# zkonduit/ezkl

Hardware: AMD Instinct MI355X
Metric: BN254 G1 MSM pts/s (2^20 points per GPU; NTT 2^22 elems/s in extra) (higher is better)
Workload: dtype u32x8 (254-bit modular integer, Montgomery); 1 GPU; configs[1]: standalone 2^20-point BN254 G1 MSM (uniform scalars, try-and-increment bases) + 2^22 scalar-field NTT per GPU; parallelism=points sharded across 1 rank(s); all_gather of 64-B partials + host fold

## Files before the change

### ezkl_amd/csrc/curve29.hpp

```cpp
#pragma once
#include "curve.hpp"
#include "field29.hpp"

namespace ezkl {

struct alignas(16) g1x29_t {
    f29_t x, y, zz, zzz;
};
struct g1a29_t {
    f29_t x, y;
};

EZ_D bool g1x29_is_id(const g1x29_t& p) { return Fq29::limbs_zero(p.zz); }
EZ_D g1x29_t g1x29_identity() {
    g1x29_t r;
    r.x = Fq29::zero(); r.y = Fq29::zero(); r.zz = Fq29::zero(); r.zzz = Fq29::zero();
    return r;
}
EZ_D g1a29_t g1a29_unpack(const g1a_t& p) {
    g1a29_t r;
    r.x = Fq29::unpack(p.x);
    r.y = Fq29::unpack(p.y);
    return r;
}
EZ_D bool g1a29_is_id(const g1a29_t& p) {
    uint32_t o = 0;
#pragma unroll
    for (int i = 0; i < 9; i++) o |= p.x.v[i] | p.y.v[i];
    return o == 0;
}

EZ_D g1x29_t g1x29_add_tail(const f29_t& u1, const f29_t& s1, const f29_t& p, const f29_t& r, const f29_t& zz, const f29_t& zzz) {
    g1x29_t o;
    const f29_t pp = Fq29::sqr(p);
    o.zz = Fq29::mul(zz, pp);
    const f29_t ppp = Fq29::mul(p, pp);
    o.zzz = Fq29::mul(zzz, ppp);
    const f29_t q = Fq29::mul(u1, pp);
#if !EZKL_FUSED_Y
    const f29_t e = Fq29::mul(s1, ppp);
#endif
    const f29_t rr = Fq29::sqr(r);
    const f29_t nq = Fq29::neg<1>(q);
    o.x = Fq29::normalize(Fq29::add(Fq29::add(rr, Fq29::neg<1>(ppp)), Fq29::add(nq, nq)));
    const f29_t d = Fq29::sub<3>(q, o.x);
#if EZKL_FUSED_Y
    o.y = Fq29::mul2add(r, d, Fq29::neg<3>(s1), ppp);
#else
    const f29_t rd = Fq29::mul(r, d);
    o.y = Fq29::normalize(Fq29::sub<1>(rd, e));
#endif
    return o;
}
EZ_D g1x29_t g1x29_double_affine(const g1a29_t& p) {
    const f29_t u = Fq29::add(p.y, p.y);
    const f29_t v = Fq29::sqr_cold(u);
    const f29_t w = Fq29::mul_cold(u, v);
    const f29_t s = Fq29::mul_cold(p.x, v);
    const f29_t xx = Fq29::sqr_cold(p.x);
    const f29_t m = Fq29::normalize(Fq29::add(Fq29::add(xx, xx), xx));
    const f29_t ns = Fq29::neg<1>(s);
    g1x29_t r;
    r.x = Fq29::normalize(Fq29::add(Fq29::sqr_cold(m), Fq29::add(ns, ns)));
    const f29_t d = Fq29::sub<3>(s, r.x);
    r.y = Fq29::normalize(Fq29::sub<1>(Fq29::mul_cold(m, d), Fq29::mul_cold(w, p.y)));
    r.zz = v;
    r.zzz = w;
    return r;
}
EZ_D g1x29_t g1x29_double(const g1x29_t& p) {
    if (g1x29_is_id(p)) return p;
    const f29_t u = Fq29::add(p.y, p.y);
    const f29_t v = Fq29::sqr_cold(u);
    const f29_t w = Fq29::mul_cold(u, v);
    const f29_t s = Fq29::mul_cold(p.x, v);
    const f29_t xx = Fq29::sqr_cold(p.x);
    const f29_t m = Fq29::normalize(Fq29::add(Fq29::add(xx, xx), xx));
    const f29_t ns = Fq29::neg<1>(s);
    g1x29_t r;
    r.x = Fq29::normalize(Fq29::add(Fq29::sqr_cold(m), Fq29::add(ns, ns)));
    const f29_t d = Fq29::sub<3>(s, r.x);
    r.y = Fq29::normalize(Fq29::sub<1>(Fq29::mul_cold(m, d), Fq29::mul_cold(w, p.y)));
    r.zz = Fq29::mul_cold(v, p.zz);
    r.zzz = Fq29::mul_cold(w, p.zzz);
    return r;
}
EZ_D g1x29_t g1x29_add_mixed(const g1x29_t& a, const g1a29_t& q, bool negate) {
    if (g1a29_is_id(q)) return a;
    const f29_t qy = negate ? Fq29::neg<0>(q.y) : q.y;
    if (g1x29_is_id(a)) {
        g1x29_t r;
        r.x = q.x;
        r.y = negate ? Fq29::normalize(qy) : q.y;
        r.zz = Fq29::one();
        r.zzz = Fq29::one();
        return r;
    }
    const f29_t u2 = Fq29::mul(q.x, a.zz);
    const f29_t s2 = Fq29::mul(qy, a.zzz);
    const f29_t p = Fq29::normalize(Fq29::sub<3>(u2, a.x));
    const f29_t r = Fq29::normalize(Fq29::sub<3>(s2, a.y));
    if (Fq29::is_zero_mod_p(p)) {
        if (Fq29::is_zero_mod_p(r)) {
            g1a29_t qq = q;
            if (negate) qq.y = Fq29::normalize(qy);
            return g1x29_double_affine(qq);
        }
        return g1x29_identity();
    }
    return g1x29_add_tail(a.x, a.y, p, r, a.zz, a.zzz);
}
EZ_D g1x29_t g1x29_add(const g1x29_t& a, const g1x29_t& b) {
    if (g1x29_is_id(a)) return b;
    if (g1x29_is_id(b)) return a;
    const f29_t u1 = Fq29::mul(a.x, b.zz), u2 = Fq29::mul(b.x, a.zz);
    const f29_t s1 = Fq29::mul(a.y, b.zzz), s2 = Fq29::mul(b.y, a.zzz);
    const f29_t p = Fq29::normalize(Fq29::sub<1>(u2, u1));
    const f29_t r = Fq29::normalize(Fq29::sub<1>(s2, s1));
    if (Fq29::is_zero_mod_p(p)) {
        if (Fq29::is_zero_mod_p(r)) return g1x29_double(a);
        return g1x29_identity();
    }
    return g1x29_add_tail(u1, s1, p, r, Fq29::mul(a.zz, b.zz), Fq29::mul(a.zzz, b.zzz));
}

EZ_D g1x29_t ld_g1x29(const g1x29_t* p) {
    g1x29_t r;
    const uint4* s = reinterpret_cast<const uint4*>(p);
    uint32_t* d = r.x.v;
#pragma unroll
    for (int k = 0; k < 9; k++) {
        const uint4 t = s[k];
        d[4 * k] = t.x; d[4 * k + 1] = t.y; d[4 * k + 2] = t.z; d[4 * k + 3] = t.w;
    }
    return r;
}
EZ_D void st_g1x29(g1x29_t* p, const g1x29_t& v) {
    uint4* d = reinterpret_cast<uint4*>(p);
    const uint32_t* s = v.x.v;
#pragma unroll
    for (int k = 0; k < 9; k++) d[k] = make_uint4(s[4 * k], s[4 * k + 1], s[4 * k + 2], s[4 * k + 3]);
}
EZ_D g1x29_t g1x29_shfl_xor(const g1x29_t& p, uint32_t mask) {
    g1x29_t r;
    const uint32_t* s = p.x.v;
    uint32_t* d = r.x.v;
#pragma unroll
    for (int k = 0; k < 36; k++) d[k] = __shfl_xor(s[k], mask);
    return r;
}
EZ_D g1x29_t g1x29_group_sum(g1x29_t acc, uint32_t width) {
#pragma unroll 1
    for (uint32_t s = width >> 1; s > 0; s >>= 1) acc = g1x29_add(acc, g1x29_shfl_xor(acc, s));
    return acc;
}

template <int S>
EZ_D f29_t f29_quad_bcast(const f29_t& x) {
    f29_t t = x, r;
    asm volatile("s_nop 1" : "+v"(t.v[0]), "+v"(t.v[1]), "+v"(t.v[2]), "+v"(t.v[3]), "+v"(t.v[4]), "+v"(t.v[5]), "+v"(t.v[6]), "+v"(t.v[7]), "+v"(t.v[8]));
#pragma unroll
    for (int i = 0; i < 9; i++) {
        r.v[i] = (uint32_t)__builtin_amdgcn_mov_dpp((int)t.v[i], S * 0x55, 0xf, 0xf, true);
        asm volatile("" : "+v"(r.v[i]));
    }
    return r;
}
EZ_D f29_t f29_sel(bool c, const f29_t& a, const f29_t& b) {
    f29_t r;
#pragma unroll
    for (int i = 0; i < 9; i++) r.v[i] = c ? a.v[i] : b.v[i];
    return r;
}
EZ_D f29_t f29_sel4(uint32_t q, const f29_t& x0, const f29_t& x1, const f29_t& x2, const f29_t& x3) {
    return f29_sel(q < 2, f29_sel(q == 0, x0, x1), f29_sel(q == 2, x2, x3));
}
template <int S>
EZ_D g1x29_t g1x29_quad_bcast(const g1x29_t& p) {
    g1x29_t r;
    r.x = f29_quad_bcast<S>(p.x); r.y = f29_quad_bcast<S>(p.y); r.zz = f29_quad_bcast<S>(p.zz); r.zzz = f29_quad_bcast<S>(p.zzz);
    return r;
}
EZ_D g1x29_t g1x29_add_quad(const g1x29_t& a, const g1x29_t& b, bool& special, uint32_t* dbg = nullptr) {
    const uint32_t q = threadIdx.x & 3u;
    g1x29_t o = a;
    special = __any(g1x29_is_id(a) || g1x29_is_id(b)) != 0;
    if (special) return o;
    const f29_t m1 = Fq29::mul(f29_sel4(q, a.x, b.x, a.y, b.y), f29_sel4(q, b.zz, a.zz, b.zzz, a.zzz));
    const f29_t u1 = f29_quad_bcast<0>(m1), s1 = f29_quad_bcast<2>(m1);
    const f29_t p = Fq29::normalize(Fq29::sub<1>(f29_quad_bcast<1>(m1), u1));
    const f29_t r = Fq29::normalize(Fq29::sub<1>(f29_quad_bcast<3>(m1), s1));
    special = __any(Fq29::is_zero_mod_p(p)) != 0;
    if (special) return o;
    const f29_t m2 = Fq29::mul(f29_sel4(q, a.zz, a.zzz, p, r), f29_sel4(q, b.zz, b.zzz, p, r));
    const f29_t pp = f29_quad_bcast<2>(m2), rr = f29_quad_bcast<3>(m2);
    const f29_t m3 = Fq29::mul(f29_sel(q == 1, p, f29_sel(q == 2, u1, m2)), pp);
    const f29_t ppp = f29_quad_bcast<1>(m3), qq = f29_quad_bcast<2>(m3);
    const f29_t nq = Fq29::neg<1>(qq);
    o.x = Fq29::normalize(Fq29::add(Fq29::add(rr, Fq29::neg<1>(ppp)), Fq29::add(nq, nq)));
    const f29_t d = Fq29::sub<3>(qq, o.x);
    const f29_t m4 = Fq29::mul(f29_sel(q == 2, r, f29_sel(q == 3, s1, m2)), f29_sel(q == 2, d, ppp));
    o.zz = f29_quad_bcast<0>(m3);
    o.zzz = f29_quad_bcast<1>(m4);
    o.y = Fq29::normalize(Fq29::sub<1>(f29_quad_bcast<2>(m4), f29_quad_bcast<3>(m4)));
    if (dbg) {
        const f29_t* t[14] = {&m1, &u1, &s1, &p, &r, &m2, &pp, &rr, &m3, &ppp, &qq, &o.x, &d, &m4};
        for (int k = 0; k < 14; k++)
            for (int i = 0; i < 9; i++) dbg[9 * k + i] = t[k]->v[i];
    }
    return o;
}
EZ_D g1x29_t g1x29_group_sum_coop(g1x29_t acc, uint32_t width) {
    const uint32_t nsteps = 3u + (31u - (uint32_t)__clz(width)) - 2u;
    g1x29_t t0 = acc;
#pragma unroll 1
    for (uint32_t k = 0; k < nsteps; k++) {
        g1x29_t a, b;
        if (k == 0) { a = g1x29_quad_bcast<0>(acc); b = g1x29_quad_bcast<1>(acc); }
        else if (k == 1) { a = g1x29_quad_bcast<2>(acc); b = g1x29_quad_bcast<3>(acc); }
        else if (k == 2) { a = t0; b = acc; }
        else { a = acc; b = g1x29_shfl_xor(acc, 4u << (k - 3u)); }
        bool special;
        g1x29_t r = g1x29_add_quad(a, b, special);
        if (special) r = g1x29_add(a, b);
        if (k == 0) t0 = r; else acc = r;
    }
    return acc;
}
EZ_D g1x29_t g1x29_block256_sum(g1x29_t acc, uint4* sh) {
    acc = g1x29_group_sum(acc, 64);
    if ((threadIdx.x & 63) == 0) {
        const uint32_t* s = acc.x.v;
#pragma unroll
        for (int k = 0; k < 9; k++) sh[k * 4 + (threadIdx.x >> 6)] = make_uint4(s[4 * k], s[4 * k + 1], s[4 * k + 2], s[4 * k + 3]);
    }
    __syncthreads();
    {
        uint32_t* d = acc.x.v;
#pragma unroll
        for (int k = 0; k < 9; k++) {
            const uint4 t = sh[k * 4 + (threadIdx.x & 3)];
            d[4 * k] = t.x; d[4 * k + 1] = t.y; d[4 * k + 2] = t.z; d[4 * k + 3] = t.w;
        }
    }
    __syncthreads();
    return g1x29_group_sum(acc, 4);
}
EZ_D g1x29_t g1x29_block256_sum_coop(const g1x29_t& acc0, uint4* sh) {
    g1x29_t acc = g1x29_group_sum_coop(acc0, 64);
    if ((threadIdx.x & 63) == 0) {
        const uint32_t* s = acc.x.v;
#pragma unroll
        for (int k = 0; k < 9; k++) sh[k * 4 + (threadIdx.x >> 6)] = make_uint4(s[4 * k], s[4 * k + 1], s[4 * k + 2], s[4 * k + 3]);
    }
    __syncthreads();
    {
        uint32_t* d = acc.x.v;
#pragma unroll
        for (int k = 0; k < 9; k++) {
            const uint4 t = sh[k * 4 + (threadIdx.x & 3)];
            d[4 * k] = t.x; d[4 * k + 1] = t.y; d[4 * k + 2] = t.z; d[4 * k + 3] = t.w;
        }
    }
    __syncthreads();
    return g1x29_group_sum(acc, 4);
}

EZ_D g1x29_t g1x29_block256_sum_coop_full(const g1x29_t& acc0, uint4* sh) {
    g1x29_t acc = g1x29_group_sum_coop(acc0, 64);
    if ((threadIdx.x & 63) == 0) {
        const uint32_t* s = acc.x.v;
#pragma unroll
        for (int k = 0; k < 9; k++) sh[k * 4 + (threadIdx.x >> 6)] = make_uint4(s[4 * k], s[4 * k + 1], s[4 * k + 2], s[4 * k + 3]);
    }
    __syncthreads();
    g1x29_t w;
    {
        uint32_t* d = w.x.v;
#pragma unroll
        for (int k = 0; k < 9; k++) {
            const uint4 t = sh[k * 4 + (threadIdx.x & 3)];
            d[4 * k] = t.x; d[4 * k + 1] = t.y; d[4 * k + 2] = t.z; d[4 * k + 3] = t.w;
        }
    }
    __syncthreads();
    return g1x29_group_sum_coop(w, 4);
}

}
```

### ezkl_amd/csrc/msm.hip

```cpp
#include "common.hpp"
#include <deque>
#include <thread>
#include <chrono>
#include "curve.hpp"
#include "curve29.hpp"
#include "host64.hpp"
#include <string.h>

namespace ezkl {

static constexpr uint32_t MSM_MAX_PART_BITS = 12;
static constexpr uint32_t MSM_SPAN_HEAVY = 16;
static constexpr uint32_t MSM_PART_STAGE = 13312;
static constexpr uint32_t MSM_BINSORT_STAGE = 15360;
static constexpr uint32_t MSM_HEAVY_CHUNK = 256;
static constexpr uint32_t MSM_DIGIT_E = 8;
static constexpr uint32_t MSM_LMIN = 8;
static constexpr uint32_t MSM_MAX_BIG = 64;
static constexpr uint32_t MSM_BIG_BLOCKS = 64;
static constexpr uint32_t MSM_BIG_ROWS = 8;

__device__ __forceinline__ uint32_t msm_part_of(uint32_t bucket, uint32_t NP) { return bucket ? 1u + (bucket & (NP - 1u)) : 0u; }
__device__ __forceinline__ uint32_t msm_lane_len(const uint32_t* offsets, uint32_t nb, uint32_t nlanes, uint32_t lmin) {
    const uint32_t l = (uint32_t)(((uint64_t)offsets[nb] + nlanes - 1) / nlanes);
// ... 203 lines not shown
    __syncthreads();
    return r;
}

__global__ __launch_bounds__(256) void msm_hist_kernel(const fe_t* scalars, size_t n, size_t per_block, WinPlan wp,
                                                       uint32_t LB, uint32_t NP, uint32_t* wg_hist, uint32_t* wg_cnt,
                                                       const fe_t* const* scal_list, uint32_t* zero_base, uint32_t zero_words, size_t bstride) {
    BOFF(); BSH(wg_hist); BSH(wg_cnt);
    if (scal_list) scalars = scal_list[blockIdx.z];
    if (zero_base) {
        BSH(zero_base);
        for (uint32_t i = blockIdx.x * 256 + threadIdx.x; i < zero_words; i += gridDim.x * 256) zero_base[i] = 0;
    }
    __shared__ uint32_t lh[(1u << MSM_MAX_PART_BITS) + 1];
    const uint32_t NQ = NP + 1;
    for (uint32_t p = threadIdx.x; p < NQ; p += 256) lh[p] = 0;
    __syncthreads();
    size_t lo = (size_t)blockIdx.x * per_block, hi = lo + per_block < n ? lo + per_block : n;
    for (size_t i0 = lo + threadIdx.x; i0 < hi; i0 += 4 * 256) {
        fe_t s[4];
        uint32_t neg[4], carry[4] = {0, 0, 0, 0};
#pragma unroll
        for (int q = 0; q < 4; q++) {
            const size_t i = i0 + (size_t)q * 256;
            if (i < hi) s[q] = msm_canon(scalars, i, neg[q]);
            else { s[q] = Fr::zero(); neg[q] = 0; }
        }
        for (uint32_t w = 0; w < wp.W; w++) {
            const uint32_t c = wp.width(w);
#pragma unroll
            for (int q = 0; q < 4; q++) {
                uint32_t bucket, sign;
                if (msm_digit_step(s[q], neg[q], c, carry[q], bucket, sign)) atomicAdd(&lh[msm_part_of(bucket, NP)], 1u);
            }
        }
    }
    __syncthreads();
    for (uint32_t p = threadIdx.x; p < NQ; p += 256) {
        wg_hist[(size_t)blockIdx.x * NQ + p] = lh[p];
        wg_cnt[(size_t)blockIdx.x * NQ + p] = lh[p];
    }
}
__global__ __launch_bounds__(1024) void msm_hist_scan_kernel(uint32_t* wg_hist, uint32_t G, uint32_t NP, uint32_t* part_count, size_t bstride) {
    BOFF(); BSH(wg_hist); BSH(part_count);
    __shared__ uint32_t sums[32][33];
    const uint32_t c = threadIdx.x & 31, j = threadIdx.x >> 5;
    const uint32_t p = blockIdx.x * 32 + c;
    const uint32_t chunk = (G + 31) / 32, g0 = j * chunk, g1 = g0 + chunk < G ? g0 + chunk : G;
    uint32_t s = 0;
    if (p < NP)
        for (uint32_t g = g0; g < g1; g++) s += wg_hist[(size_t)g * NP + p];
    sums[j][c] = s;
    __syncthreads();
    if (j == 0) {
        uint32_t run = 0;
        for (uint32_t q = 0; q < 32; q++) {
            uint32_t v = sums[q][c];
            sums[q][c] = run;
            run += v;
        }
        if (p < NP) part_count[p] = run;
    }
    __syncthreads();
    if (p < NP) {
        uint32_t run = sums[j][c];
        for (uint32_t g = g0; g < g1; g++) {
            uint32_t v = wg_hist[(size_t)g * NP + p];
            wg_hist[(size_t)g * NP + p] = run;
            run += v;
        }
    }
}
__device__ __forceinline__ void msm_part_scan_body(const uint32_t* part_count, uint32_t NQ, uint32_t* part_base, uint32_t* big_flag,
                                                   uint32_t* big_list, uint32_t* big_count, uint32_t* sh) {
    const uint32_t t = threadIdx.x;
    constexpr uint32_t PER = 5;
    uint32_t v[PER], sum = 0;
#pragma unroll
    for (uint32_t q = 0; q < PER; q++) {
        const uint32_t i = PER * t + q;
        v[q] = i < NQ ? part_count[i] : 0;
        sum += v[q];
    }
    uint32_t total;
    uint32_t run = msm_block_scan(sum, sh, total) - sum;
#pragma unroll
    for (uint32_t q = 0; q < PER; q++) {
        const uint32_t i = PER * t + q;
        if (i < NQ) part_base[i] = run;
        run += v[q];
    }
    if (t == 1023) part_base[NQ] = total;
#pragma unroll
    for (uint32_t q = 0; q < PER; q++) {
        const uint32_t i = PER * t + q;
        if (i == 0 || i >= NQ) continue;
        uint32_t slot = 0;
        if (v[q] > MSM_BINSORT_STAGE) {
            slot = atomicAdd(big_count, 1u);
            if (slot < MSM_MAX_BIG) big_list[slot] = i - 1;
            slot = slot < MSM_MAX_BIG ? slot + 1 : 0;
        }
        big_flag[i - 1] = slot;
    }
}
__global__ __launch_bounds__(1024) void msm_part_scan_kernel(const uint32_t* part_count, uint32_t NQ, uint32_t* part_base, uint32_t* big_flag,
                                                             uint32_t* big_list, uint32_t* big_count, size_t bstride) {
    BOFF(); BSH(part_count); BSH(part_base); BSH(big_flag); BSH(big_list); BSH(big_count);
    __shared__ uint32_t sh[1024];
    msm_part_scan_body(part_count, NQ, part_base, big_flag, big_list, big_count, sh);
}
__global__ __launch_bounds__(1024) void msm_partition_kernel(const fe_t* scalars, size_t n, size_t per_block, WinPlan wp,
                                                             uint32_t LB, uint32_t NP, size_t base_offset, size_t tab_stride,
                                                             const uint32_t* part_base, const uint32_t* wg_hist, const uint32_t* wg_cnt, uint2* entries,
                                                             uint32_t* vals, const fe_t* const* scal_list, size_t bstride) {
    BOFF(); BSH(part_base); BSH(wg_hist); BSH(wg_cnt); BSH(entries); BSH(vals);
    if (scal_list) scalars = scal_list[blockIdx.z];
    extern __shared__ uint32_t plds[];
    __shared__ uint32_t tsum[1024];
    const uint32_t NQ = NP + 1;
    uint32_t* start = plds;
    uint32_t* cursor = plds + (NQ + 1);
    uint32_t* gbase = plds + 2 * (NQ + 1);
    uint2* stage = reinterpret_cast<uint2*>(plds + 3 * (NQ + 1));
    const uint32_t t = threadIdx.x, T = blockDim.x;
    const uint32_t K = (NQ + T - 1) / T;
    uint32_t loc = 0;
    for (uint32_t q = 0; q < K; q++) {
        const uint32_t p = t * K + q;
        if (p < NQ) loc += wg_cnt[(size_t)blockIdx.x * NQ + p];
    }
    uint32_t total;
    uint32_t run = msm_block_scan(loc, tsum, total) - loc;
    for (uint32_t q = 0; q < K; q++) {
        const uint32_t p = t * K + q;
        if (p < NQ) {
            start[p] = run;
            cursor[p] = run;
            gbase[p] = part_base[p] + wg_hist[(size_t)blockIdx.x * NQ + p];
            run += wg_cnt[(size_t)blockIdx.x * NQ + p];
        }
    }
    __syncthreads();
    const size_t lo = (size_t)blockIdx.x * per_block, hi = lo + per_block < n ? lo + per_block : n;
    const size_t i = lo + t;
    if (i < hi) {
        uint32_t neg;
        fe_t s = msm_canon(scalars, i, neg);
        msm_foreach_digit(s, neg, wp, [&](uint32_t w, uint32_t bucket, uint32_t sign) {
            const uint32_t r = atomicAdd(&cursor[msm_part_of(bucket, NP)], 1u);
            stage[r] = make_uint2((uint32_t)(w * tab_stride + base_offset + i) | (sign << 31), bucket);
        });
    }
    __syncthreads();
    const uint32_t PB = 31 - __clz(NP);
    for (uint32_t idx = t; idx < total; idx += T) {
        const uint2 e = stage[idx];
        const uint32_t p = msm_part_of(e.y, NP);
        const uint32_t slot = gbase[p] + (idx - start[p]);
        if (p) entries[slot] = make_uint2(e.x, e.y >> PB);
        else vals[slot] = e.x;
    }
}
__device__ __forceinline__ uint32_t msm_wave_rank(uint32_t* cnt, uint32_t key) {
    const uint64_t active = __ballot(1);
    const uint32_t first = __builtin_amdgcn_readfirstlane(key);
    if (__ballot(key == first) == active) {
        const uint32_t rank = (uint32_t)__popcll(active & ((1ull << (threadIdx.x & 63u)) - 1ull));
        uint32_t base = 0;
        if (rank == 0) base = atomicAdd(&cnt[first], (uint32_t)__popcll(active));
        return (uint32_t)__builtin_amdgcn_readfirstlane(base) + rank;
    }
    return atomicAdd(&cnt[key], 1u);
}
__device__ __forceinline__ void msm_bins_scan(uint32_t* cnt, uint32_t* tsum, uint32_t nbins, uint32_t p, uint32_t beg, const uint32_t* part_base,
                                              bool emit, uint32_t* offsets, g1x29_t* buckets) {
    const uint32_t t = threadIdx.x;
    uint32_t loc[4], s = 0;
#pragma unroll
    for (int q = 0; q < 4; q++) {
        uint32_t j = t * 4 + q;
        loc[q] = j < nbins ? cnt[j] : 0;
        s += loc[q];
    }
    uint32_t total;
    uint32_t run = msm_block_scan(s, tsum, total) - s;
#pragma unroll
    for (int q = 0; q < 4; q++) {
        uint32_t j = t * 4 + q;
        if (j < nbins) {
            cnt[j] = run;
            if (emit) {
                const bool b0 = (p == 0 && j == 0);
                offsets[(size_t)p * nbins + j] = b0 ? part_base[0] : beg + run;
                if (b0 ? part_base[1] == part_base[0] : loc[q] == 0) st_f29(&buckets[(size_t)p * nbins + j].zz, Fq29::zero());
            }
        }
        run += loc[q];
    }
    __syncthreads();
}
__device__ __forceinline__ void msm_bigsort_count_body(const uint2* entries, const uint32_t* part_base, uint32_t LB, const uint32_t* big_list,
                                                       const uint32_t* big_count, uint32_t* bin_total, uint32_t* block_off, uint32_t* cnt, uint32_t bx,
                                                       uint32_t by, uint32_t rows);
__global__ __launch_bounds__(512) void msm_binsort_kernel(const uint2* entries, const uint32_t* part_base, uint32_t LB, uint32_t NP,
                                                          const uint32_t* big_flag, uint32_t* offsets, uint32_t* vals, g1x29_t* buckets,
                                                          const uint32_t* big_list, const uint32_t* big_count, uint32_t* bin_total, uint32_t* block_off,
                                                          size_t bstride) {
    BOFF(); BSH(entries); BSH(part_base); BSH(big_flag); BSH(offsets); BSH(vals); BSH(buckets);
    __shared__ uint32_t cnt[2048];
    __shared__ uint32_t tsum[512];
    extern __shared__ uint32_t stage[];
    if (blockIdx.x >= NP) {
        BSH(big_list); BSH(big_count); BSH(bin_total); BSH(block_off);
        const uint32_t w = blockIdx.x - NP;
        msm_bigsort_count_body(entries, part_base, LB, big_list, big_count, bin_total, block_off, cnt, w % MSM_BIG_BLOCKS, w / MSM_BIG_BLOCKS, MSM_BIG_ROWS);
        return;
    }
    const uint32_t p = blockIdx.x, t = threadIdx.x, nbins = 1u << LB;
    const uint32_t beg = part_base[p + 1], end = part_base[p + 2];
    if (p == NP - 1 && t == 0) offsets[(size_t)NP * nbins] = end;
    if (big_flag[p]) return;
    const bool staged = (end - beg) <= MSM_BINSORT_STAGE;
    for (uint32_t j = t; j < nbins; j += 512) cnt[j] = 0;
    __syncthreads();
    if (staged) {
        constexpr int PER = MSM_BINSORT_STAGE / 512;
        uint2 v[PER];
#pragma unroll
        for (int q = 0; q < PER; q++) {
            const uint32_t e = beg + t + (uint32_t)q * 512u;
            v[q] = e < end ? entries[e] : make_uint2(0u, 0xffffffffu);
        }
#pragma unroll
        for (int q = 0; q < PER; q++)
            if (v[q].y != 0xffffffffu) atomicAdd(&cnt[v[q].y], 1u);
        __syncthreads();
        msm_bins_scan(cnt, tsum, nbins, p, beg, part_base, true, offsets, buckets);
#pragma unroll
        for (int q = 0; q < PER; q++)
            if (v[q].y != 0xffffffffu) stage[atomicAdd(&cnt[v[q].y], 1u)] = v[q].x;
        __syncthreads();
        for (uint32_t i = t; i < end - beg; i += 512) vals[beg + i] = stage[i];
    } else {
        for (uint32_t e = beg + t; e < end; e += 512) (void)msm_wave_rank(cnt, entries[e].y);
        __syncthreads();
        msm_bins_scan(cnt, tsum, nbins, p, beg, part_base, true, offsets, buckets);
        for (uint32_t e = beg + t; e < end; e += 512) {
            const uint2 v = entries[e];
            vals[beg + msm_wave_rank(cnt, v.y)] = v.x;
        }
    }
}
__device__ __forceinline__ void msm_big_slice(uint32_t beg, uint32_t end, uint32_t& s0, uint32_t& s1, uint32_t bx) {
    const uint32_t chunk = (end - beg + MSM_BIG_BLOCKS - 1) / MSM_BIG_BLOCKS;
    s0 = beg + bx * chunk;
    s1 = s0 + chunk < end ? s0 + chunk : end;
    if (s0 > end) s0 = end;
}
__device__ __forceinline__ void msm_bigsort_count_body(const uint2* entries, const uint32_t* part_base, uint32_t LB, const uint32_t* big_list,
                                                       const uint32_t* big_count, uint32_t* bin_total, uint32_t* block_off, uint32_t* cnt, uint32_t bx,
                                                       uint32_t by, uint32_t rows) {
    const uint32_t t = threadIdx.x, nbins = 1u << LB;
    const uint32_t nbig = big_count[0] < MSM_MAX_BIG ? big_count[0] : MSM_MAX_BIG;
    for (uint32_t y = by; y < nbig; y += rows) {
        const uint32_t p = big_list[y];
        uint32_t s0, s1;
        msm_big_slice(part_base[p + 1], part_base[p + 2], s0, s1, bx);
        for (uint32_t j = t; j < nbins; j += 512) cnt[j] = 0;
        __syncthreads();
        for (uint32_t e = s0 + t; e < s1; e += 512) (void)msm_wave_rank(cnt, entries[e].y);
        __syncthreads();
        for (uint32_t j = t; j < nbins; j += 512)
            block_off[((size_t)y * MSM_BIG_BLOCKS + bx) * nbins + j] = cnt[j] ? atomicAdd(&bin_total[(size_t)y * nbins + j], cnt[j]) : 0u;
        __syncthreads();
    }
}
__global__ __launch_bounds__(512) void msm_bigsort_scatter_kernel(const uint2* entries, const uint32_t* part_base, uint32_t LB, const uint32_t* big_list,
                                                                  const uint32_t* big_count, const uint32_t* bin_total, const uint32_t* block_off,
                                                                  uint32_t* offsets, uint32_t* vals, g1x29_t* buckets, size_t bstride) {
    BOFF(); BSH(entries); BSH(part_base); BSH(big_list); BSH(big_count); BSH(bin_total); BSH(block_off); BSH(offsets); BSH(vals); BSH(buckets);
    __shared__ uint32_t cnt[2048];
    __shared__ uint32_t tsum[512];
    const uint32_t t = threadIdx.x, nbins = 1u << LB;
    const uint32_t nbig = big_count[0] < MSM_MAX_BIG ? big_count[0] : MSM_MAX_BIG;
    for (uint32_t y = blockIdx.y; y < nbig; y += gridDim.y) {
        const uint32_t p = big_list[y], beg = part_base[p + 1];
        uint32_t s0, s1;
        msm_big_slice(beg, part_base[p + 2], s0, s1, blockIdx.x);
        for (uint32_t j = t; j < nbins; j += 512) cnt[j] = bin_total[(size_t)y * nbins + j];
        __syncthreads();
        msm_bins_scan(cnt, tsum, nbins, p, beg, part_base, blockIdx.x == 0, offsets, buckets);
        const uint32_t* mine = block_off + ((size_t)y * MSM_BIG_BLOCKS + blockIdx.x) * nbins;
        for (uint32_t j = t; j < nbins; j += 512) cnt[j] += mine[j];
        __syncthreads();
        for (uint32_t e = s0 + t; e < s1; e += 512) {
            const uint2 v = entries[e];
            vals[beg + msm_wave_rank(cnt, v.y)] = v.x;
        }
        __syncthreads();
    }
}

struct MsmRec {
    g1a_t p;
    bool neg;
};
__device__ __forceinline__ MsmRec msm_fetch(const g1a_t* tab, uint32_t v) {
    MsmRec r;
    r.p = ld_g1a(tab + (v & 0x7fffffffu));
    r.neg = (v >> 31) != 0;
    return r;
}
__global__ __launch_bounds__(256, 3) void msm_accumulate_kernel(const g1a_t* tab, const uint32_t* offsets, const uint32_t* vals,
                                                             uint32_t nb, uint32_t nlanes, g1x29_t* buckets, g1x29_t* head, g1x29_t* tail,
                                                             uint32_t* lane_first, uint32_t lmin, size_t bstride) {
    BOFF(); BSH(offsets); BSH(vals); BSH(buckets); BSH(head); BSH(tail); BSH(lane_first);
    const uint32_t t = blockIdx.x * blockDim.x + threadIdx.x;
    const uint32_t total = offsets[nb], L = msm_lane_len(offsets, nb, nlanes, lmin);
    const uint64_t k0w = (uint64_t)t * L;
    if (k0w >= total) return;
    const uint32_t k0 = (uint32_t)k0w;
    const uint32_t k1 = (uint64_t)k0 + L < total ? k0 + L : total;
    uint32_t lo = 0, hi = nb;
    while (hi - lo > 1) {
        uint32_t mid = (lo + hi) >> 1;
        if (offsets[mid] <= k0) lo = mid; else hi = mid;
    }
    uint32_t b = lo, bin_end = offsets[b + 1];
    uint32_t end_next = offsets[b + 2 <= nb ? b + 2 : nb];
    lane_first[t] = b;
    bool started_before = offsets[b] < k0;
    g1x29_t acc = g1x29_identity();
    MsmRec nxt = msm_fetch(tab, vals[k0]);
    uint32_t vn = k0 + 1 < k1 ? vals[k0 + 1] : 0u;
    for (uint32_t k = k0; k < k1; k++) {
        if (k == bin_end) {
            if (started_before) st_g1x29(head + t, acc); else st_g1x29(buckets + b, acc);
            acc.zz = Fq29::zero();
            started_before = false;
            b++;
            bin_end = end_next;
            if (bin_end == k) {
                uint32_t probes = 1;
                while (bin_end == k && probes < 4) { b++; bin_end = offsets[b + 1]; probes++; }
                if (bin_end == k) {
                    uint32_t lo2 = b + 1, hi2 = nb;
                    while (hi2 - lo2 > 1) {
                        uint32_t mid = (lo2 + hi2) >> 1;
                        if (offsets[mid] <= k) lo2 = mid; else hi2 = mid;
                    }
                    b = lo2;
                    bin_end = offsets[b + 1];
                }
            }
            end_next = offsets[b + 2 <= nb ? b + 2 : nb];
        }
        const MsmRec cur = nxt;
        nxt = msm_fetch(tab, vn);
        vn = k + 2 < k1 ? vals[k + 2] : 0u;
        acc = g1x29_add_mixed(acc, g1a29_unpack(cur.p), cur.neg);
    }
    if (k1 == bin_end) {
        if (started_before) st_g1x29(head + t, acc); else st_g1x29(buckets + b, acc);
    } else {
        if (started_before) st_g1x29(head + t, acc); else st_g1x29(tail + t, acc);
    }
}
EZ_D g1x29_t g1x29_shfl_down(const g1x29_t& p, uint32_t d) {
    g1x29_t r;
    const uint32_t* s = p.x.v;
    uint32_t* o = r.x.v;
#pragma unroll
    for (int k = 0; k < 36; k++) o[k] = __shfl_down(s[k], d);
    return r;
}
__global__ __launch_bounds__(256) void msm_fixup_boundary_tree_kernel(const uint32_t* offsets, uint32_t nb, uint32_t nlanes,
                                                                      const uint32_t* lane_first, const g1x29_t* head, const g1x29_t* tail, g1x29_t* buckets,
                                                                      uint32_t* heavy_list, uint32_t* heavy_count, uint32_t* chunk_list, uint32_t lmin,
                                                                      uint32_t span_heavy, size_t bstride) {
    BOFF(); BSH(offsets); BSH(lane_first); BSH(head); BSH(tail); BSH(buckets); BSH(heavy_list); BSH(heavy_count); BSH(chunk_list);
    const uint32_t t = blockIdx.x * blockDim.x + threadIdx.x + 1;
    const uint32_t lane = threadIdx.x & 63u;
    const uint32_t L = msm_lane_len(offsets, nb, nlanes, lmin);
    const uint64_t k0 = (uint64_t)t * L;
    bool cut = t < nlanes && k0 < offsets[nb];
    uint32_t b = 0, t1 = 0, t2 = 0;
    if (cut) {
        b = lane_first[t];
        const uint32_t beg = offsets[b], end = offsets[b + 1];
        cut = beg < k0;
        t1 = beg / L; t2 = (end - 1) / L;
    }
    if (cut && t2 - t1 > span_heavy) {
        if (t == t1 + 1 && t2 - t1 > MSM_HEAVY_CHUNK) heavy_list[atomicAdd(heavy_count, 1u)] = b;
        if ((t - t1 - 1) % MSM_HEAVY_CHUNK == 0) chunk_list[atomicAdd(heavy_count + 1, 1u)] = t;
        cut = false;
    }
    const uint32_t wave_last = t + (63u - lane);
    const uint32_t run = cut ? (t2 < wave_last ? t2 : wave_last) - t + 1u : 0u;
    uint32_t longest = run;
#pragma unroll
    for (uint32_t o = 32; o > 0; o >>= 1) {
        const uint32_t m = __shfl_xor(longest, o);
        longest = m > longest ? m : longest;
    }
    if (longest == 0) return;
    if (longest <= 2) {
        if (!cut || t != t1 + 1) return;
        g1x29_t acc = g1x29_add(ld_g1x29(tail + t1), ld_g1x29(head + t));
        for (uint32_t u = t + 1; u <= t2; u++) acc = g1x29_add(acc, ld_g1x29(head + u));
        st_g1x29(buckets + b, acc);
        return;
    }
    g1x29_t v = cut ? ld_g1x29(head + t) : g1x29_identity();
    uint32_t have = cut ? 1u : 0u;
#pragma unroll 1
    for (uint32_t d = 1; d < longest; d <<= 1) {
        const g1x29_t w = g1x29_shfl_down(v, d);
        const uint32_t hw = __shfl_down(have, d);
        if (have == d && run > d) {
            v = g1x29_add(v, w);
            have += hw;
        }
    }
    if (!cut || t != t1 + 1) return;
    g1x29_t acc = g1x29_add(ld_g1x29(tail + t1), v);
    for (uint32_t u = t + run; u <= t2; u++) acc = g1x29_add(acc, ld_g1x29(head + u));
    st_g1x29(buckets + b, acc);
}
__global__ __launch_bounds__(256) void msm_fixup_heavy1_kernel(const uint32_t* offsets, uint32_t nb, uint32_t nlanes, const uint32_t* lane_first, g1x29_t* head,
                                                               const g1x29_t* tail, g1x29_t* buckets, const uint32_t* chunk_list, const uint32_t* counts, uint32_t lmin,
                                                               uint32_t coop, size_t bstride) {
    BOFF(); BSH(offsets); BSH(lane_first); BSH(head); BSH(tail); BSH(buckets); BSH(chunk_list); BSH(counts);
    const uint32_t nchunks = counts[1], L = msm_lane_len(offsets, nb, nlanes, lmin);
    const uint32_t wave = threadIdx.x >> 6, lane = threadIdx.x & 63u;
    for (uint32_t ci = blockIdx.x * 4u + wave; ci < nchunks; ci += gridDim.x * 4u) {
        const uint32_t start = chunk_list[ci], b = lane_first[start];
        const uint32_t t2 = (offsets[b + 1] - 1) / L;
        const uint32_t stop = start + MSM_HEAVY_CHUNK - 1 < t2 ? start + MSM_HEAVY_CHUNK - 1 : t2;
        const uint32_t t1 = offsets[b] / L;
        const bool whole = t2 - t1 <= MSM_HEAVY_CHUNK;
        g1x29_t acc = (whole && lane == 63u) ? ld_g1x29(tail + t1) : g1x29_identity();
        for (uint32_t t = start + lane; t <= stop; t += 64) acc = g1x29_add(acc, ld_g1x29(head + t));
        acc = coop ? g1x29_group_sum_coop(acc, 64) : g1x29_group_sum(acc, 64);
        if (lane == 0) st_g1x29(whole ? buckets + b : head + start, acc);
    }
}
__global__ __launch_bounds__(256) void msm_fixup_heavy2_kernel(const uint32_t* offsets, uint32_t nb, uint32_t nlanes, const g1x29_t* head, const g1x29_t* tail,
                                                               const uint32_t* heavy_list, const uint32_t* counts, g1x29_t* buckets, uint32_t lmin, uint32_t coop, size_t bstride) {
    BOFF(); BSH(offsets); BSH(head); BSH(tail); BSH(heavy_list); BSH(counts); BSH(buckets);
    const uint32_t L = msm_lane_len(offsets, nb, nlanes, lmin);
    const uint32_t wave = threadIdx.x >> 6, lane = threadIdx.x & 63u;
    for (uint32_t h = blockIdx.x * 4u + wave; h < counts[0]; h += gridDim.x * 4u) {
        const uint32_t b = heavy_list[h];
        const uint32_t t1 = offsets[b] / L, t2 = (offsets[b + 1] - 1) / L;
        g1x29_t acc = lane == 63u ? ld_g1x29(tail + t1) : g1x29_identity();
        for (uint32_t t = t1 + 1 + lane * MSM_HEAVY_CHUNK; t <= t2; t += 64 * MSM_HEAVY_CHUNK) acc = g1x29_add(acc, ld_g1x29(head + t));
        acc = coop ? g1x29_group_sum_coop(acc, 64) : g1x29_group_sum(acc, 64);
        if (lane == 0) st_g1x29(buckets + b, acc);
    }
}

struct ReduceGeom {
    uint32_t wA, wB, wC;
    uint32_t wsA, wsB, wsC;
    uint32_t EA, GA, ET, GT;
};
__global__ __launch_bounds__(256, 2) void msm_reduce1_kernel(const g1x29_t* buckets, ReduceGeom g, g1x29_t* partA, g1x29_t* partT, size_t bstride) {
    BOFF(); BSH(buckets); BSH(partA); BSH(partT);
    const uint32_t idx = blockIdx.x * blockDim.x + threadIdx.x;
    g1x29_t acc = g1x29_identity();
    if (blockIdx.y == 0) {
        if (idx >= (g.GA << g.wA)) return;
        const uint32_t dA = idx & ((1u << g.wA) - 1u), grp = idx >> g.wA;
        for (uint32_t e = 0; e < g.EA; e++) acc = g1x29_add(acc, ld_g1x29(buckets + ((((size_t)grp * g.EA + e) << g.wA) | dA)));
        st_g1x29(partA + (size_t)dA * g.GA + grp, acc);
    } else {
        const uint32_t nT = 1u << (g.wB + g.wC);
        if (idx >= nT * g.GT) return;
        const uint32_t grp = idx % g.GT, t = idx / g.GT;
        for (uint32_t e = 0; e < g.ET; e++) acc = g1x29_add(acc, ld_g1x29(buckets + (((size_t)t << g.wA) | (e * g.GT + grp))));
        st_g1x29(partT + (size_t)t * g.GT + grp, acc);
    }
}
__global__ __launch_bounds__(64) void msm_reduce2_kernel(const g1x29_t* partA, const g1x29_t* partT, ReduceGeom g, g1x29_t* SA, g1x29_t* T, uint32_t lanesA,
                                                         uint32_t lanesT, uint32_t blocksA, uint32_t coop, size_t bstride) {
    BOFF(); BSH(partA); BSH(partT); BSH(SA); BSH(T);
    const bool isA = blockIdx.x < blocksA;
    const uint32_t lanes = isA ? lanesA : lanesT, per = 64 / lanes;
    const uint32_t o = (isA ? blockIdx.x : blockIdx.x - blocksA) * per + threadIdx.x / lanes, j = threadIdx.x % lanes;
    const uint32_t nout = isA ? (1u << g.wA) : (1u << (g.wB + g.wC)), G = isA ? g.GA : g.GT;
    g1x29_t acc = g1x29_identity();
    if (o < nout) {
        const g1x29_t* src = (isA ? partA : partT) + (size_t)o * G;
        for (uint32_t i = j; i < G; i += lanes) acc = g1x29_add(acc, ld_g1x29(src + i));
    }
    acc = (coop && lanes >= 4) ? g1x29_group_sum_coop(acc, lanes) : g1x29_group_sum(acc, lanes);
    if (j == 0 && o < nout) st_g1x29((isA ? SA : T) + o, acc);
}
__global__ __launch_bounds__(256) void msm_planes_kernel(const g1x29_t* SA, const g1x29_t* T, ReduceGeom g, g1x29_t* planes, g1x29_t* planes_host, uint32_t coop,
                                                         size_t bstride) {
    BOFF(); BSH(SA); BSH(T); BSH(planes);
    __shared__ uint4 sh[9 * 4];
    uint32_t id = blockIdx.x, field = 0, j = 0;
    if (id > 0) {
        id -= 1;
        if (id < g.wA) { field = 1; j = id; }
        else if (id < g.wA + g.wB) { field = 2; j = id - g.wA; }
        else { field = 3; j = id - g.wA - g.wB; }
    }
    const uint32_t nA = 1u << g.wA, nT = 1u << (g.wB + g.wC);
    g1x29_t acc = g1x29_identity();
    auto with_bit = [](uint32_t k, uint32_t bit) { return ((k >> bit) << (bit + 1)) | (1u << bit) | (k & ((1u << bit) - 1u)); };
    if (field == 0) {
        for (uint32_t d = threadIdx.x; d < nA; d += 256) acc = g1x29_add(acc, ld_g1x29(SA + d));
    } else if (field == 1) {
        for (uint32_t k = threadIdx.x; k < nA / 2; k += 256) acc = g1x29_add(acc, ld_g1x29(SA + with_bit(k, j)));
    } else {
        const uint32_t sh_bits = field == 2 ? j : g.wB + j;
        for (uint32_t k = threadIdx.x; k < nT / 2; k += 256) acc = g1x29_add(acc, ld_g1x29(T + with_bit(k, sh_bits)));
    }
    acc = (coop & 8u) ? g1x29_block256_sum_coop_full(acc, sh) : coop ? g1x29_block256_sum_coop(acc, sh) : g1x29_block256_sum(acc, sh);
    if (threadIdx.x == 0) {
        const uint32_t ws = field == 1 ? g.wsA : field == 2 ? g.wsB : g.wsC;
        const uint32_t slot = field == 0 ? 0u : 1u + ws + j;
        st_g1x29(planes + slot, acc);
        if (planes_host) st_g1x29(planes_host + (size_t)blockIdx.z * 32 + slot, acc);
    }
}

static int table_build(Ctx* c, hipStream_t st, const Bases* b, bool wait) {
    MsmTable t;
    t.n = b->n;
    t.wp = pick_plan(b->n);
    if ((size_t)t.wp.W * t.n >= ((size_t)1 << 31)) return EZKL_ERR_UNSUPPORTED;
    EZ_HIP(hipMalloc(&t.tab, (size_t)t.wp.W * t.n * sizeof(g1a_t)));
    EZ_HIP(hipMemcpyAsync(t.tab, b->pts, t.n * sizeof(g1a_t), hipMemcpyDeviceToDevice, st));
    for (uint32_t w = 1; w < t.wp.W; w++)
        hipLaunchKernelGGL(msm_precompute_kernel, dim3(cdiv(t.n, 256)), dim3(256), 0, st, t.tab + (size_t)(w - 1) * t.n,
                           t.tab + (size_t)w * t.n, t.n, t.wp.width(w - 1));
    hipLaunchKernelGGL(msm_table_to_r261_kernel, dim3(cdiv((size_t)t.wp.W * t.n, 256)), dim3(256), 0, st, t.tab, (size_t)t.wp.W * t.n);
    EZ_HIP(hipGetLastError());
    EZ_HIP(hipEventCreateWithFlags(&t.ready, hipEventDisableTiming));
    EZ_HIP(hipEventRecord(t.ready, st));
    if (wait) {
        EZ_HIP(hipStreamSynchronize(st));
        t.synced = true;
    }
    g_tables[b] = t;
    return EZKL_OK;
}
static int table_get(Ctx* c, hipStream_t st, const Bases* b, MsmTable** out) {
    auto it = g_tables.find(b);
    if (it == g_tables.end()) {
        int rc = table_build(c, st, b, true);
        if (rc) return rc;
        it = g_tables.find(b);
    }
    if (!it->second.synced) {
        EZ_HIP(hipEventSynchronize(it->second.ready));
        it->second.synced = true;
    }
    *out = &it->second;
    return EZKL_OK;
}
int msm_table_prepare(Ctx* c, const Bases* b) {
    if (g_tables.count(b)) return EZKL_OK;
    if (!g_table_stream) EZ_HIP(hipStreamCreateWithFlags(&g_table_stream, hipStreamNonBlocking));
    return table_build(c, g_table_stream, b, false);
}
void msm_table_drop(const Bases* b) {
    auto it = g_tables.find(b);
    if (it != g_tables.end()) {
        if (it->second.ready) { (void)hipEventSynchronize(it->second.ready); (void)hipEventDestroy(it->second.ready); }
        (void)hipFree(it->second.tab);
        g_tables.erase(it);
    }
}

static constexpr size_t MSM_MAX_GROUP = 16;
static int slot_prepare(MsmSlot& sl, size_t bytes, size_t msms = 1) {
    if (!sl.st) {
        EZ_HIP(stream_create_prio(&sl.st, "EZKL_HIP_PRIO_MSM", 0));
        EZ_HIP(hipEventCreateWithFlags(&sl.done, hipEventDisableTiming));
        EZ_HIP(hipHostMalloc((void**)&sl.list_pinned, MSM_MAX_GROUP * sizeof(void*), hipHostMallocDefault));
    }
    if (msms > sl.pinned_msms) {
        if (sl.pinned) {
            EZ_HIP(hipStreamSynchronize(sl.st));
            EZ_HIP(hipHostFree(sl.pinned));
            sl.pinned = nullptr;
        }
        EZ_HIP(hipHostMalloc((void**)&sl.pinned, msms * 32 * sizeof(g1x29_t), hipHostMallocDefault));
        EZ_HIP(hipHostGetDevicePointer(&sl.pinned_dev, sl.pinned, 0));
        sl.pinned_msms = msms;
    }
    if (bytes > sl.scratch_bytes) {
        if (sl.scratch) {
            EZ_HIP(hipStreamSynchronize(sl.st));
            EZ_HIP(hipFree(sl.scratch));
            sl.scratch = nullptr;
            sl.scratch_bytes = 0;
        }
        size_t want = bytes + (bytes >> 4);
        EZ_HIP(hipMalloc((void**)&sl.scratch, want));
        sl.scratch_bytes = want;
    }
    return EZKL_OK;
}
static int msm_finish(MsmSlot& sl, void* out_host = nullptr, bool release = true) {
    if (!out_host) out_host = sl.out;
    EZ_HIP(hipEventSynchronize(sl.done));
    for (uint32_t j = 0; j < sl.count; j++) {
        const uint32_t* hp = sl.pinned + (size_t)j * 32 * 36;
        h64::xyzz acc = h64::identity();
        for (int k = (int)sl.bits - 1; k >= 0; k--) {
            acc = h64::dbl(acc);
            acc = h64::add(acc, h64::from_limbs29_point(hp + 36 * (1 + k)));
        }
        acc = h64::add(acc, h64::from_limbs29_point(hp));
        h64::aff r = h64::to_affine(acc);
        memcpy((uint8_t*)out_host + 64 * (size_t)j, &r, 64);
    }
    if (release) sl.busy = false;
    return EZKL_OK;
}

static size_t msm_group_size(const MsmTable* T, size_t n, bool small_scalars, size_t batch = 0) {
    if (const char* e = getenv("EZKL_MSM_GROUP")) {
        const int v = atoi(e);
        if (v >= 1 && v <= (int)MSM_MAX_GROUP) return (size_t)v;
    }
    (void)T; (void)n; (void)batch;
    if (small_scalars) {
        static const int small = [] { const char* e = getenv("EZKL_MSM_GROUP_SMALL"); const int v = e ? atoi(e) : 0; return v >= 1 && v <= (int)MSM_MAX_GROUP ? v : 6; }();
        return (size_t)small;
    }
    static const int big = [] { const char* e = getenv("EZKL_MSM_GROUP_BIG"); const int v = e ? atoi(e) : 0; return v >= 1 && v <= (int)MSM_MAX_GROUP ? v : 4; }();
    return (size_t)big;
}
static int msm_enqueue(Ctx* c, MsmSlot& sl, hipStream_t st, MsmTable* T, size_t base_offset, const fe_t* const* cols, size_t count, size_t n, bool timed) {
    int rc = EZKL_OK;
    if (count < 1 || count > MSM_MAX_GROUP) return EZKL_ERR_INVALID;
    const unsigned Z = (unsigned)count;
    const fe_t* scalars = cols[0];
    const WinPlan wp = T->wp;
    const uint32_t W = wp.W, bits = wp.cmax() - 1;
    const uint32_t nb = 1u << bits;
    const size_t npairs = n * W;
    uint32_t PB = bits < 10 ? bits : 10;
    while (PB < bits && PB < MSM_MAX_PART_BITS && (npairs >> PB) > (size_t)MSM_BINSORT_STAGE * 9 / 10) PB++;
    const uint32_t LB = bits - PB, NP = 1u << PB;
    int& acc_blocks_per_cu = msm_state().acc_blocks_per_cu;
    if (!acc_blocks_per_cu) {
        EZ_HIP(hipFuncSetAttribute((const void*)msm_binsort_kernel, hipFuncAttributeMaxDynamicSharedMemorySize, 96 * 1024));
        EZ_HIP(hipFuncSetAttribute((const void*)msm_partition_kernel, hipFuncAttributeMaxDynamicSharedMemorySize, 144 * 1024));
        EZ_HIP(hipOccupancyMaxActiveBlocksPerMultiprocessor(&acc_blocks_per_cu, msm_accumulate_kernel, 256, 0));
        if (acc_blocks_per_cu < 1) acc_blocks_per_cu = 1;
    }
    const size_t resident = (size_t)acc_blocks_per_cu * 256 * c->num_cus;
    const size_t load = npairs >> bits, per_lane = load * 9 / 10 > 40 ? load * 9 / 10 : 40;
    size_t rounds = npairs / (resident * per_lane);
    if (rounds < 1) rounds = 1;
    uint32_t L = (uint32_t)((npairs + resident * rounds - 1) / (resident * rounds));
    if (L < 8) L = 8;
    if (const char* e = getenv("EZKL_MSM_L")) {
        const int v = atoi(e);
        if (v > 0 && v < (1 << 20)) L = (uint32_t)v;
    }
// ... 642 lines not shown
```

Before: 807.3 million pts/s.

## Spill bucket zz/zzz to LDS and prefetch bases via global_load_lds in accumulate

The MSM accumulate kernel now keeps only the affine-like x/y accumulator in registers and moves the zz/zzz coordinates into per-thread LDS slots, read and written with inline ds_read/ds_write asm. The next base point is prefetched straight into LDS with global_load_lds instead of into registers. The mixed add is split into head and tail parts so the prefetch issues between them. Together these cut VGPR pressure so launch bounds can rise from 3 to 4 waves, hiding more latency, at the cost of extra LDS traffic, manual waitcnt fences and fragile inline assembly.

```diff
diff --git a/ezkl_amd/csrc/curve29.hpp b/ezkl_amd/csrc/curve29.hpp
--- a/ezkl_amd/csrc/curve29.hpp
+++ b/ezkl_amd/csrc/curve29.hpp
@@ -52,18 +52,20 @@
 #endif
     return o;
 }
+template <bool COLD = true>
 EZ_D g1x29_t g1x29_double_affine(const g1a29_t& p) {
+    auto mul = [](const f29_t& a, const f29_t& b) { return COLD ? Fq29::mul_cold(a, b) : Fq29::mul(a, b); };
     const f29_t u = Fq29::add(p.y, p.y);
-    const f29_t v = Fq29::sqr_cold(u);
-    const f29_t w = Fq29::mul_cold(u, v);
-    const f29_t s = Fq29::mul_cold(p.x, v);
-    const f29_t xx = Fq29::sqr_cold(p.x);
+    const f29_t v = mul(u, u);
+    const f29_t w = mul(u, v);
+    const f29_t s = mul(p.x, v);
+    const f29_t xx = mul(p.x, p.x);
     const f29_t m = Fq29::normalize(Fq29::add(Fq29::add(xx, xx), xx));
     const f29_t ns = Fq29::neg<1>(s);
     g1x29_t r;
-    r.x = Fq29::normalize(Fq29::add(Fq29::sqr_cold(m), Fq29::add(ns, ns)));
+    r.x = Fq29::normalize(Fq29::add(mul(m, m), Fq29::add(ns, ns)));
     const f29_t d = Fq29::sub<3>(s, r.x);
-    r.y = Fq29::normalize(Fq29::sub<1>(Fq29::mul_cold(m, d), Fq29::mul_cold(w, p.y)));
+    r.y = Fq29::normalize(Fq29::sub<1>(mul(m, d), mul(w, p.y)));
     r.zz = v;
     r.zzz = w;
     return r;
diff --git a/ezkl_amd/csrc/msm.hip b/ezkl_amd/csrc/msm.hip
--- a/ezkl_amd/csrc/msm.hip
+++ b/ezkl_amd/csrc/msm.hip
@@ -529,21 +529,134 @@
     }
 }
 
-struct MsmRec {
-    g1a_t p;
-    bool neg;
+struct MsmAccLds {
+    uint4 rec[4][4][64];
+    uint4 zq[4][256];
+    uint32_t z8[2][256];
 };
-__device__ __forceinline__ MsmRec msm_fetch(const g1a_t* tab, uint32_t v) {
-    MsmRec r;
-    r.p = ld_g1a(tab + (v & 0x7fffffffu));
-    r.neg = (v >> 31) != 0;
+static_assert(sizeof(MsmAccLds) == 34816, "accumulate kernel: 136 bytes of LDS per lane");
+struct MsmAccZ {
+    uint32_t zq, z8;
+};
+typedef uint32_t u32x4_t __attribute__((ext_vector_type(4)));
+typedef __attribute__((address_space(3))) void* lds_ptr_t;
+EZ_D MsmAccZ msm_acc_z(MsmAccLds& sh, uint32_t tid) {
+    MsmAccZ z;
+    z.zq = (uint32_t)(uintptr_t)(lds_ptr_t)&sh.zq[0][tid];
+    z.z8 = (uint32_t)(uintptr_t)(lds_ptr_t)&sh.z8[0][tid];
+    return z;
+}
+EZ_D void msm_lds_fence() { asm volatile("" ::: "memory"); }
+template <int WHICH>
+EZ_D f29_t msm_ld_z(const MsmAccZ& z) {
+    u32x4_t a, b;
+    f29_t r;
+    asm volatile("ds_read_b128 %0, %3 offset:%5\n\tds_read_b128 %1, %3 offset:%6\n\tds_read_b32 %2, %4 offset:%7\n\ts_waitcnt lgkmcnt(0)"
+                 : "=&v"(a), "=&v"(b), "=&v"(r.v[8])
+                 : "v"(z.zq), "v"(z.z8), "i"(WHICH * 8192), "i"(WHICH * 8192 + 4096), "i"(WHICH * 1024)
+                 : "memory");
+    r.v[0] = a.x; r.v[1] = a.y; r.v[2] = a.z; r.v[3] = a.w;
+    r.v[4] = b.x; r.v[5] = b.y; r.v[6] = b.z; r.v[7] = b.w;
     return r;
 }
-__global__ __launch_bounds__(256, 3) void msm_accumulate_kernel(const g1a_t* tab, const uint32_t* offsets, const uint32_t* vals,
+template <int WHICH>
+EZ_D void msm_st_z(const MsmAccZ& z, const f29_t& v) {
+    u32x4_t a, b;
+    a.x = v.v[0]; a.y = v.v[1]; a.z = v.v[2]; a.w = v.v[3];
+    b.x = v.v[4]; b.y = v.v[5]; b.z = v.v[6]; b.w = v.v[7];
+    asm volatile("ds_write_b128 %0, %2 offset:%5\n\tds_write_b128 %0, %3 offset:%6\n\tds_write_b32 %1, %4 offset:%7\n\ts_nop 1"
+                 :
+                 : "v"(z.zq), "v"(z.z8), "v"(a), "v"(b), "v"(v.v[8]), "i"(WHICH * 8192), "i"(WHICH * 8192 + 4096), "i"(WHICH * 1024)
+                 : "memory");
+}
+typedef const __attribute__((address_space(1))) uint32_t* gu32_ptr_t;
+EZ_D void msm_fetch_lds(const g1a_t* tab, uint32_t v, uint4 (*slot)[64]) {
+    typedef const __attribute__((address_space(1))) void* gptr_t;
+    const char* src = reinterpret_cast<const char*>(tab + (v & 0x7fffffffu));
+    msm_lds_fence();
+#pragma unroll
+    for (int j = 0; j < 4; j++) __builtin_amdgcn_global_load_lds((gptr_t)(src + 16 * j), (lds_ptr_t)&slot[j][0], 16, 0, 0);
+    msm_lds_fence();
+}
+EZ_D g1a_t msm_ld_rec(const uint4 (*slot)[64], uint32_t lane) {
+    g1a_t r;
+    const uint4 a = slot[0][lane], b = slot[1][lane], c = slot[2][lane], d = slot[3][lane];
+    r.x.v[0] = a.x; r.x.v[1] = a.y; r.x.v[2] = a.z; r.x.v[3] = a.w; r.x.v[4] = b.x; r.x.v[5] = b.y; r.x.v[6] = b.z; r.x.v[7] = b.w;
+    r.y.v[0] = c.x; r.y.v[1] = c.y; r.y.v[2] = c.z; r.y.v[3] = c.w; r.y.v[4] = d.x; r.y.v[5] = d.y; r.y.v[6] = d.z; r.y.v[7] = d.w;
+    return r;
+}
+EZ_D bool msm_add_head(f29_t& ax, f29_t& ay, const MsmAccZ& z, const g1a29_t& q, bool negate, f29_t& p, f29_t& r) {
+    if (g1a29_is_id(q)) return false;
+    const f29_t qy = negate ? Fq29::neg<0>(q.y) : q.y;
+    const f29_t zz = msm_ld_z<0>(z);
+    if (Fq29::limbs_zero(zz)) {
+        ax = q.x;
+        ay = negate ? Fq29::normalize(qy) : q.y;
+        msm_st_z<0>(z, Fq29::one());
+        msm_st_z<1>(z, Fq29::one());
+        return false;
+    }
+    const f29_t u2 = Fq29::mul(q.x, zz);
+    const f29_t s2 = Fq29::mul(qy, msm_ld_z<1>(z));
+    p = Fq29::normalize(Fq29::sub<3>(u2, ax));
+    r = Fq29::normalize(Fq29::sub<3>(s2, ay));
+    if (Fq29::is_zero_mod_p(p)) {
+        if (Fq29::is_zero_mod_p(r)) {
+            g1a29_t qq = q;
+            if (negate) qq.y = Fq29::normalize(qy);
+            const g1x29_t d = g1x29_double_affine<false>(qq);
+            ax = d.x; ay = d.y;
+            msm_st_z<0>(z, d.zz);
+            msm_st_z<1>(z, d.zzz);
+        } else {
+            msm_st_z<0>(z, Fq29::zero());
+        }
+        return false;
+    }
+    return true;
+}
+EZ_D void msm_add_tail(f29_t& ax, f29_t& ay, const MsmAccZ& z, const f29_t& p, const f29_t& r) {
+    const f29_t pp = Fq29::sqr(p);
+    msm_st_z<0>(z, Fq29::mul(msm_ld_z<0>(z), pp));
+    const f29_t ppp = Fq29::mul(p, pp);
+    msm_st_z<1>(z, Fq29::mul(msm_ld_z<1>(z), ppp));
+    const f29_t q = Fq29::mul(ax, pp);
+#if !EZKL_FUSED_Y
+    const f29_t e = Fq29::mul(ay, ppp);
+#endif
+    const f29_t rr = Fq29::sqr(r);
+    const f29_t nq = Fq29::neg<1>(q);
+    const f29_t x3 = Fq29::normalize(Fq29::add(Fq29::add(rr, Fq29::neg<1>(ppp)), Fq29::add(nq, nq)));
+    const f29_t d = Fq29::sub<3>(q, x3);
+#if EZKL_FUSED_Y
+    ay = Fq29::mul2add(r, d, Fq29::neg<3>(ay), ppp);
+#else
+    ay = Fq29::normalize(Fq29::sub<1>(Fq29::mul(r, d), e));
+#endif
+    ax = x3;
+}
+EZ_D void msm_st_acc(g1x29_t* dst, const f29_t& ax, const f29_t& ay, const MsmAccZ& z) {
+    g1x29_t o;
+    o.x = ax; o.y = ay; o.zz = msm_ld_z<0>(z); o.zzz = msm_ld_z<1>(z);
+    __attribute__((address_space(1))) u32x4_t* d = (__attribute__((address_space(1))) u32x4_t*)dst;
+    const uint32_t* s = o.x.v;
+#pragma unroll
+    for (int k = 0; k < 9; k++) {
+        u32x4_t w;
+        w.x = s[4 * k]; w.y = s[4 * k + 1]; w.z = s[4 * k + 2]; w.w = s[4 * k + 3];
+        d[k] = w;
+    }
+}
+__global__ __launch_bounds__(256, 4) void msm_accumulate_kernel(const g1a_t* tab, const uint32_t* offsets, const uint32_t* vals,
                                                              uint32_t nb, uint32_t nlanes, g1x29_t* buckets, g1x29_t* head, g1x29_t* tail,
                                                              uint32_t* lane_first, uint32_t lmin, size_t bstride) {
+    __shared__ MsmAccLds sh;
     BOFF(); BSH(offsets); BSH(vals); BSH(buckets); BSH(head); BSH(tail); BSH(lane_first);
-    const uint32_t t = blockIdx.x * blockDim.x + threadIdx.x;
+    const uint32_t tid = threadIdx.x, lane = tid & 63u;
+    uint4 (*slot)[64] = sh.rec[tid >> 6];
+    const MsmAccZ z = msm_acc_z(sh, tid);
+    const gu32_ptr_t goffsets = (gu32_ptr_t)offsets, gvals = (gu32_ptr_t)vals;
+    const uint32_t t = blockIdx.x * blockDim.x + tid;
     const uint32_t total = offsets[nb], L = msm_lane_len(offsets, nb, nlanes, lmin);
     const uint64_t k0w = (uint64_t)t * L;
     if (k0w >= total) return;
@@ -554,45 +667,52 @@
         uint32_t mid = (lo + hi) >> 1;
         if (offsets[mid] <= k0) lo = mid; else hi = mid;
     }
-    uint32_t b = lo, bin_end = offsets[b + 1];
-    uint32_t end_next = offsets[b + 2 <= nb ? b + 2 : nb];
+    uint32_t b = lo, bin_end = goffsets[b + 1];
+    uint32_t end_next = goffsets[b + 2 <= nb ? b + 2 : nb];
     lane_first[t] = b;
-    bool started_before = offsets[b] < k0;
-    g1x29_t acc = g1x29_identity();
-    MsmRec nxt = msm_fetch(tab, vals[k0]);
-    uint32_t vn = k0 + 1 < k1 ? vals[k0 + 1] : 0u;
+    bool started_before = goffsets[b] < k0;
+    f29_t ax = Fq29::zero(), ay = Fq29::zero();
+    msm_st_z<0>(z, Fq29::zero());
+    msm_st_z<1>(z, Fq29::zero());
+    uint32_t vc = gvals[k0];
+    msm_fetch_lds(tab, vc, slot);
+    uint32_t vn = k0 + 1 < k1 ? gvals[k0 + 1] : 0u;
     for (uint32_t k = k0; k < k1; k++) {
+        asm volatile("s_waitcnt vmcnt(0)" ::: "memory");
+        const g1a_t cur = msm_ld_rec(slot, lane);
+        const bool neg = (vc >> 31) != 0;
         if (k == bin_end) {
-            if (started_before) st_g1x29(head + t, acc); else st_g1x29(buckets + b, acc);
-            acc.zz = Fq29::zero();
+            msm_st_acc(started_before ? head + t : buckets + b, ax, ay, z);
+            msm_st_z<0>(z, Fq29::zero());
             started_before = false;
             b++;
             bin_end = end_next;
             if (bin_end == k) {
                 uint32_t probes = 1;
-                while (bin_end == k && probes < 4) { b++; bin_end = offsets[b + 1]; probes++; }
+                while (bin_end == k && probes < 4) { b++; bin_end = goffsets[b + 1]; probes++; }
                 if (bin_end == k) {
                     uint32_t lo2 = b + 1, hi2 = nb;
                     while (hi2 - lo2 > 1) {
                         uint32_t mid = (lo2 + hi2) >> 1;
-                        if (offsets[mid] <= k) lo2 = mid; else hi2 = mid;
+                        if (goffsets[mid] <= k) lo2 = mid; else hi2 = mid;
                     }
                     b = lo2;
-                    bin_end = offsets[b + 1];
+                    bin_end = goffsets[b + 1];
                 }
             }
-            end_next = offsets[b + 2 <= nb ? b + 2 : nb];
-        }
-        const MsmRec cur = nxt;
-        nxt = msm_fetch(tab, vn);
-        vn = k + 2 < k1 ? vals[k + 2] : 0u;
-        acc = g1x29_add_mixed(acc, g1a29_unpack(cur.p), cur.neg);
-    }
-    if (k1 == bin_end) {
-        if (started_before) st_g1x29(head + t, acc); else st_g1x29(buckets + b, acc);
-    } else {
-        if (started_before) st_g1x29(head + t, acc); else st_g1x29(tail + t, acc);
-    }
+            end_next = goffsets[b + 2 <= nb ? b + 2 : nb];
+        }
+        f29_t p, r;
+        const bool general = msm_add_head(ax, ay, z, g1a29_unpack(cur), neg, p, r);
+        asm volatile("s_waitcnt lgkmcnt(0)" ::: "memory");
+        msm_fetch_lds(tab, vn, slot);
+        vc = vn;
+        vn = k + 2 < k1 ? gvals[k + 2] : 0u;
+        if (general) msm_add_tail(ax, ay, z, p, r);
+        msm_lds_fence();
+    }
+    g1x29_t* dst = started_before ? head + t : k1 == bin_end ? buckets + b : tail + t;
+    msm_st_acc(dst, ax, ay, z);
 }
 EZ_D g1x29_t g1x29_shfl_down(const g1x29_t& p, uint32_t d) {
     g1x29_t r;
```

Result: no change. 807.1 million pts/s (-0.0%).
